# jlogan03/interpn

Hardware: AMD Instinct MI355X
Metric: Mpoints/sec (f64) per GPU + achieved HBM GB/s vs roofline, 3D linear-regular (higher is better)
Workload: dtype f64

## Files before the change

interpn_amd/csrc/abi_binned.hip:

```cpp
#include "abi_internal.h"

using namespace interpn;
using namespace interpn_abi;

namespace interpn_abi {


size_t bin_slice_points(const GridDesc& g) {
  const int lg = g.cfg.bin_slice_log2 >= 16 && g.cfg.bin_slice_log2 <= 27 ? g.cfg.bin_slice_log2 : 25;
  const size_t s = (size_t)1 << lg;
  return s < kBinSlicePoints ? s : kBinSlicePoints;
}

int binned_applies(const GridDesc& g, size_t npoints) {
  if (g.method != kCubic || !g.bricks || g.ndims < 2 || g.ndims > 4) return 0;
  if (g.cfg.binned == 0 || g.cfg.force_generic) return 1;
  const bool main11 = g.brick_step[0] == 1 && g.brick_step[1] == 1;
  const bool second = !main11 && g.bricks11 != nullptr;
  if (g.cfg.binned < 0) {
    if (g.ndims != 4 && g.ndims != 3) return 0;
    if (!main11 && !second) return 0;
    if (g.ndims == 3) return 0;
    if (main11) {
      unsigned nb[2];
      size_t table = 0;
      cubic_tile_geometry(g, 1, 1, nb, &table);
      if (table <= thresholds(g.cfg).binned_table_min) return 0;
    }
    if (npoints < thresholds(g.cfg).binned_points_min) return 1;
  }
  return 2;
}

interpn_hip_interp::BinSlot* take_bin_slot(interpn_hip_interp* h, size_t need, hipStream_t stream, bool may_alloc, int* why) {
  using Slot = interpn_hip_interp::BinSlot;
  std::unique_lock<std::mutex> lk(h->bin_mu);
  Slot* pick = nullptr;
  bool wait = false;
  for (auto& sl : h->bin_slots)
    if (!sl.busy && sl.bytes >= need && sl.recorded && sl.last_stream == stream) { pick = &sl; break; }
  if (!pick)
    for (auto& sl : h->bin_slots) {
      if (sl.busy || sl.bytes < need) continue;
      if (!sl.recorded) { pick = &sl; break; }
      const hipError_t q = hipEventQuery(sl.event);
      if (q == hipSuccess) { pick = &sl; break; }
      if (q != hipErrorNotReady) (void)hipGetLastError();
    }
  if (!pick && may_alloc && h->bin_slots.size() < interpn_hip_interp::kMaxBinSlots) {
    Slot sl;
    if (hipEventCreateWithFlags(&sl.event, hipEventDisableTiming) != hipSuccess) { (void)hipGetLastError(); *why = INTERPN_HIP_WHY_ALLOC_FAILED; return nullptr; }
    if (pool_alloc(h->device, &sl.scratch, need) != hipSuccess) {
      (void)hipGetLastError();
      (void)hipEventDestroy(sl.event);
      *why = INTERPN_HIP_WHY_ALLOC_FAILED;
      return nullptr;
    }
    sl.bytes = need;
    h->scratch_allocs.fetch_add(1);
    h->bin_slots.push_back(sl);
    pick = &h->bin_slots.back();
  }
  if (!pick) {
    for (auto& sl : h->bin_slots)
      if (!sl.busy && sl.bytes >= need && (!pick || sl.stamp < pick->stamp)) pick = &sl;
    wait = pick != nullptr;
  }
  if (!pick && may_alloc) {
    for (auto& sl : h->bin_slots)
      if (!sl.busy && (!pick || sl.stamp < pick->stamp)) pick = &sl;
    if (pick) {
      pick->busy = true;
      const bool recorded = pick->recorded;
      const hipEvent_t ev = pick->event;
      void* const old = pick->scratch;
      lk.unlock();
      bool freed = false;
      void* fresh = nullptr;
      bool ok = !recorded || hipEventSynchronize(ev) == hipSuccess;
      if (ok) {
        pool_free(h->device, old);
        freed = true;
        ok = pool_alloc(h->device, &fresh, need) == hipSuccess;
      }
      if (!ok) (void)hipGetLastError();
      lk.lock();
      if (freed) h->sampling.last_word = nullptr;
      pick->busy = false;
      if (!ok) {
        if (freed) { pick->scratch = nullptr; pick->bytes = 0; pick->recorded = false; }
        pick->totals_clean = false;
        pick->sweep_clean = false;
        *why = INTERPN_HIP_WHY_ALLOC_FAILED;
        return nullptr;
      }
      pick->scratch = fresh;
      pick->bytes = need;
      pick->totals_clean = false;
      pick->sweep_clean = false;
      pick->recorded = false;
      h->scratch_allocs.fetch_add(1);
    }
  }
  if (!pick) { *why = INTERPN_HIP_WHY_NO_SCRATCH; return nullptr; }
  if (wait && pick->recorded && pick->last_stream != stream &&
      hipStreamWaitEvent(stream, pick->event, 0) != hipSuccess) { (void)hipGetLastError(); *why = INTERPN_HIP_WHY_NO_SCRATCH; return nullptr; }
  if (!wait && pick->recorded && pick->last_stream != stream) (void)hipStreamWaitEvent(stream, pick->event, 0);
  pick->busy = true;
  pick->stamp = ++h->bin_uses;
  return pick;
}

void release_bin_slot(interpn_hip_interp* h, interpn_hip_interp::BinSlot* slot, hipStream_t stream, bool staged) {
  std::lock_guard<std::mutex> lk(h->bin_mu);
  if (hipEventRecord(slot->event, stream) == hipSuccess) {
    slot->recorded = true;
  } else {
    (void)hipGetLastError();
    (void)hipStreamSynchronize(stream);
    slot->recorded = false;
  }
  slot->last_stream = stream;
  slot->busy = false;
  slot->staged = staged;
}

int eval_device_binned(interpn_hip_interp* h, const void* const* obs, void* out, size_t npoints, hipStream_t stream,
                       unsigned flags, int* why) {
  const GridDesc& g = h->desc;
  *why = INTERPN_HIP_WHY_NONE;
  const int applies = binned_applies(g, npoints);
  if (applies < 2) { *why = applies ? INTERPN_HIP_WHY_SMALL_OR_OFF : INTERPN_HIP_WHY_NONE; return -1; }
  const bool main11 = g.brick_step[0] == 1 && g.brick_step[1] == 1;
  const bool second = !main11 && g.bricks11 != nullptr;
  GridDesc second_desc;
  const GridDesc* use = &g;
  if (second) {
    second_desc = g;
    second_desc.bricks = g.bricks11;
    second_desc.brick_step[0] = second_desc.brick_step[1] = 1;
    second_desc.brick_nb[0] = g.bricks11_nb[0];
    second_desc.brick_nb[1] = g.bricks11_nb[1];
    use = &second_desc;
  }
  BinPlan plan;
  bool column3_go = false;
  bool column = g.cfg.column != 0 && (second || main11) && cubic_column_applies(*use);
  const bool column3 = g.ndims == 3 && g.cfg.column != 0 && (second || main11) && cubic3_column_applies(*use);
  if (g.ndims == 3 && g.cfg.binned < 0 && !column3) { *why = INTERPN_HIP_WHY_NONE; return -1; }
  {
    const size_t slice_max0 = bin_slice_points(g);
    const size_t per_slice = npoints < slice_max0 ? npoints : slice_max0;
    ColumnPlan cp0;
    size_t per_bin_min = 2304;
// ... 161 lines not shown
  if (!h || !ms || n < 4) return INTERPN_HIP_ERR_INVALID_ARGUMENT;
  DeviceGuard guard(h->device);
  if (!guard.ok()) return INTERPN_HIP_ERR_NO_DEVICE;
  std::lock_guard<std::mutex> lk(h->bin_mu);
  const interpn_hip_interp::BinSlot* best = nullptr;
  for (const auto& sl : h->bin_slots)
    if (sl.staged && !sl.busy && (!best || sl.stamp > best->stamp)) best = &sl;
  if (!best) return INTERPN_HIP_ERR_INVALID_ARGUMENT;
  HIP_TRY(hipEventSynchronize(best->stage[4]));
  for (int k = 0; k < 4; ++k) {
    float f = 0.f;
    HIP_TRY(hipEventElapsedTime(&f, best->stage[k], best->stage[k + 1]));
    ms[k] = (double)f;
  }
  return INTERPN_HIP_OK;
}

int interpn_hip_reserve(interpn_hip_interp* h, size_t npoints, int nstreams) {
  if (!h || nstreams < 0) return INTERPN_HIP_ERR_INVALID_ARGUMENT;
  if ((size_t)nstreams > interpn_hip_interp::kMaxBinSlots) nstreams = (int)interpn_hip_interp::kMaxBinSlots;
  const GridDesc& g = h->desc;
  const bool sorts = binned_applies(g, npoints) >= 2, sweeps = sweep_applies(g, npoints) >= 2;
  if (npoints == 0 || nstreams == 0 || (!sorts && !sweeps)) return INTERPN_HIP_OK;
  DeviceGuard guard(h->device);
  if (!guard.ok()) return INTERPN_HIP_ERR_NO_DEVICE;
  const size_t slice_max = bin_slice_points(g);
  const size_t need = sorts ? bin_scratch_bytes(g, npoints < slice_max ? npoints : slice_max) : sweep_work_bytes();
  std::lock_guard<std::mutex> lk(h->bin_mu);
  int have = 0;
  for (auto& sl : h->bin_slots)
    if (sl.bytes >= need) ++have;
  for (auto& sl : h->bin_slots) {
    if (have >= nstreams) break;
    if (sl.bytes >= need || sl.busy) continue;
    if (sl.recorded) HIP_TRY(hipEventSynchronize(sl.event));
    pool_free(h->device, sl.scratch);
    h->sampling.last_word = nullptr;
    sl.scratch = nullptr;
    sl.bytes = 0;
    sl.totals_clean = false;
    sl.sweep_clean = false;
    sl.recorded = false;
    hipError_t e = pool_alloc(h->device, &sl.scratch, need);
    if (e != hipSuccess) { (void)hipGetLastError(); sl.scratch = nullptr; return INTERPN_HIP_ERR_OUT_OF_MEMORY; }
    sl.bytes = need;
    h->scratch_allocs.fetch_add(1);
    ++have;
  }
  while (have < nstreams && h->bin_slots.size() < interpn_hip_interp::kMaxBinSlots) {
    interpn_hip_interp::BinSlot sl;
    HIP_TRY(hipEventCreateWithFlags(&sl.event, hipEventDisableTiming));
    hipError_t e = pool_alloc(h->device, &sl.scratch, need);
    if (e != hipSuccess) { (void)hipGetLastError(); (void)hipEventDestroy(sl.event); return INTERPN_HIP_ERR_OUT_OF_MEMORY; }
    sl.bytes = need;
    h->scratch_allocs.fetch_add(1);
    h->bin_slots.push_back(sl);
    ++have;
  }
  return have >= nstreams ? INTERPN_HIP_OK : INTERPN_HIP_ERR_OUT_OF_MEMORY;
}

}
```

interpn_amd/csrc/abi_create.hip:

```cpp
#include "abi_internal.h"
#include "cubic_cell_record.h"

using namespace interpn;
using namespace interpn_abi;

namespace interpn_abi {

thread_local bool t_defer_tables = false;

int finish_create(interpn_hip_interp* h, const void* vals, size_t nvals, size_t elem, int vals_mem) {
  GridDesc& g = h->desc;
  {
    const DeviceProps dp = device_props(h->device);
    g.cfg.num_cus = dp.num_cus;
    g.cfg.num_xcds = dp.num_xcds;
    g.cfg.l2_bytes = dp.l2_bytes;
    g.cfg.lds_per_cu = dp.lds_per_cu;
    g.cfg.lds_per_wg = dp.lds_per_wg;
  }
  latch_env(g.cfg);
  g.nvals = nvals;
  if (vals_mem == INTERPN_HIP_MEM_DEVICE) {
    g.vals = vals;
  } else {
// ... 477 lines not shown
  const size_t elem = g.dtype == kF64 ? 8 : 4;
  hipError_t e = pool_alloc(dev, &h->vals_owned, g.nvals * elem);
  if (e == hipSuccess) e = hipMemcpyPeer(h->vals_owned, dev, src->desc.vals, src->device, g.nvals * elem);
  if (e == hipSuccess && src->desc.axis_image && g.axis_alloc_bytes) {
    e = pool_alloc(dev, &h->grids_owned, g.axis_alloc_bytes);
    if (e == hipSuccess) e = hipMemcpyPeer(h->grids_owned, dev, src->desc.axis_image, src->device, g.axis_alloc_bytes);
    if (e == hipSuccess) {
      g.axis_image = h->grids_owned;
      for (int d = 0; d < g.ndims; ++d) g.grid[d] = (const char*)h->grids_owned + g.axis_g_off[d];
    }
  }
  if (e != hipSuccess) {
    interpn_hip_destroy(h);
    return hip_fail(e);
  }
  st = finish_create(h, h->vals_owned, g.nvals, elem, INTERPN_HIP_MEM_DEVICE);
  if (st) {
    interpn_hip_destroy(h);
    return st;
  }
  *out = h;
  return INTERPN_HIP_OK;
}

int interpn_hip_elem_size(const interpn_hip_interp* h) { return h ? (h->desc.dtype == kF64 ? 8 : 4) : 0; }
int interpn_hip_ndims(const interpn_hip_interp* h) { return h ? h->desc.ndims : 0; }
int interpn_hip_device(const interpn_hip_interp* h) { return h ? h->device : -1; }

void interpn_hip_destroy(interpn_hip_interp* h) {
  if (!h) return;
  DeviceGuard guard(h->device);
  {
    std::lock_guard<std::mutex> lk(h->marks_mu);
    for (auto& m : h->marks) {
      if (hipEventSynchronize(m.event) != hipSuccess) { (void)hipGetLastError(); h->sync_device_at_destroy = true; }
      (void)hipEventDestroy(m.event);
    }
    h->marks.clear();
  }
  for (auto& l : h->lane)
    if (l.stream && hipStreamSynchronize(l.stream) != hipSuccess) { (void)hipGetLastError(); h->sync_device_at_destroy = true; }
  if (h->sync_device_at_destroy) (void)hipDeviceSynchronize();
  for (auto& l : h->lane) {
    if (l.stream) pool_return_kit(h->device, l.stream, l.flag_host);
    pool_free(h->device, l.flag_dev);
    pool_free(h->device, l.obs);
    pool_free(h->device, l.out);
  }
  pool_return_small(h->device, h->small_host);
  for (auto& sl : h->bin_slots) {
    if (sl.event) (void)hipEventDestroy(sl.event);
    for (hipEvent_t e : sl.stage)
      if (e) (void)hipEventDestroy(e);
    pool_free(h->device, sl.scratch);
  }
  pool_free(h->device, h->first_bad);
  pool_return_pinned_word(h->device, h->finish_word);
  pool_return_pinned_word(h->device, h->sampling.host);
  pool_free(h->device, h->grids_owned);
  pool_free(h->device, h->bricks_owned);
  pool_free(h->device, h->bricks11_owned);
  pool_free(h->device, h->sweep_owned);
  pool_free(h->device, h->vals_owned);
  delete h;
}

}
```

interpn_amd/csrc/abi_fields.hip:

```cpp
#include <climits>

#include "abi_internal.h"

using namespace interpn;
using namespace interpn_abi;

namespace {

struct DeferTables {
  explicit DeferTables(bool on) { t_defer_tables = on; }
  ~DeferTables() { t_defer_tables = false; }
};

long long env_number(const char* name, long long fallback) {
  const char* env = getenv(name);
  if (!env || !*env) return fallback;
  char* end = nullptr;
  const long long v = strtoll(env, &end, 0);
  return (end == env || *end != 0) ? fallback : v;
}

}

namespace interpn_abi {
// ... 281 lines not shown
        [&](int m, size_t prod) { return validate_rectilinear<T>(m, grids, grid_lens, ngrids, prod); },               \
        [&](const T* v, size_t prod, int dev, interpn_hip_interp** h) {                                               \
          return create_rectilinear<T>(method, grids, grid_lens, ngrids, v, prod, INTERPN_HIP_MEM_DEVICE,             \
                                       linearize_extrapolation, dev, h);                                              \
        });                                                                                                           \
  }
DEFINE_FIELDS(double, f64)
DEFINE_FIELDS(float, f32)

int interpn_hip_fields_eval_device(interpn_hip_fields* s, const void* const* obs, size_t nobs, void* out, size_t out_stride,
                                   size_t npoints, void* stream, unsigned flags, int* path_taken) {
  if (path_taken) *path_taken = INTERPN_HIP_FIELDS_PATH_PER_FIELD;
  if (!s || s->sub.empty() || (!obs && nobs)) return INTERPN_HIP_ERR_INVALID_ARGUMENT;
  if (flags & ~(unsigned)INTERPN_HIP_EVAL_NO_ALLOC) return INTERPN_HIP_ERR_INVALID_ARGUMENT;
  int st = validate_obs(s->sub[0]->desc, nullptr, nobs, npoints);
  if (st) return st;
  if (npoints == 0) return INTERPN_HIP_OK;
  if (!out || out_stride < npoints) return INTERPN_HIP_ERR_INVALID_ARGUMENT;
  for (size_t i = 0; i < nobs; ++i)
    if (!obs[i]) return INTERPN_HIP_ERR_INVALID_ARGUMENT;
  DeviceGuard guard(s->device);
  if (!guard.ok()) return INTERPN_HIP_ERR_NO_DEVICE;
  hipStream_t hs = static_cast<hipStream_t>(stream);
  const bool fused = columns_take_fused(s, npoints, hs, flags);
  st = eval_columns(s, fused, obs, out, out_stride, npoints, hs, flags);
  if (st == INTERPN_HIP_OK && fused && path_taken) *path_taken = INTERPN_HIP_FIELDS_PATH_FUSED;
  return st;
}

int interpn_hip_fields_finish(interpn_hip_fields* s, void* stream, uint64_t* first_bad_index) {
  if (!s || s->sub.empty()) return INTERPN_HIP_ERR_INVALID_ARGUMENT;
  const size_t count = s->per_field_pending ? s->nfields : 1;
  s->per_field_pending = false;
  int error = INTERPN_HIP_OK;
  uint64_t best = ~(uint64_t)0;
  for (size_t f = 0; f < count; ++f) {
    uint64_t bad = 0;
    const int st = interpn_hip_finish(s->sub[f], stream, &bad);
    if (st == s->sub[f]->desc.unrep_status) best = bad < best ? bad : best;
    else if (st != INTERPN_HIP_OK && error == INTERPN_HIP_OK) error = st;
  }
  if (error) return error;
  if (best != ~(uint64_t)0) {
    if (first_bad_index) *first_bad_index = best;
    return s->sub[0]->desc.unrep_status;
  }
  return INTERPN_HIP_OK;
}

int interpn_hip_fields_eval_host(interpn_hip_fields* s, const void* const* obs, const size_t* obs_lens, size_t nobs, void* out,
                                 size_t out_stride, size_t nout) {
  if (!s || s->sub.empty() || (!obs && nobs) || (!obs_lens && nobs)) return INTERPN_HIP_ERR_INVALID_ARGUMENT;
  int st = validate_obs(s->sub[0]->desc, obs_lens, nobs, nout);
  if (st) return st;
  if (nout == 0) return INTERPN_HIP_OK;
  if (!out || out_stride < nout) return INTERPN_HIP_ERR_INVALID_ARGUMENT;
  for (size_t i = 0; i < nobs; ++i)
    if (!obs[i]) return INTERPN_HIP_ERR_INVALID_ARGUMENT;
  DeviceGuard guard(s->device);
  if (!guard.ok()) return INTERPN_HIP_ERR_NO_DEVICE;
  const size_t elem = s->dtype == kF64 ? 8 : 4;
  const long long opt_chunk = s->sub[0]->desc.cfg.host_chunk;
  size_t chunk = opt_chunk >= 1 ? (size_t)opt_chunk : ((size_t)2 << 20);
  if (chunk > nout) chunk = nout;
  std::lock_guard<std::mutex> host_lock(s->host_mu);
  if (!s->stream) HIP_TRY(pool_take_kit(s->device, &s->stream, &s->kit_word));
// ... 187 lines not shown
```

interpn_amd/csrc/abi_host.hip:

```cpp
#include "abi_internal.h"

using namespace interpn;
using namespace interpn_abi;

namespace interpn_abi {

int ensure_lane(interpn_hip_interp* h, int which, size_t points) {
  interpn_hip_interp::HostLane& l = h->lane[which];
  if (l.points >= points && l.obs) return INTERPN_HIP_OK;
  const size_t elem = h->desc.dtype == kF64 ? 8 : 4;
  if (l.obs) { HIP_TRY(hipStreamSynchronize(l.stream)); pool_free(h->device, l.obs); l.obs = nullptr; }
  if (l.out) { pool_free(h->device, l.out); l.out = nullptr; }
  l.points = 0;
  if (!l.stream) HIP_TRY(pool_take_kit(h->device, &l.stream, &l.flag_host));
  HIP_TRY(pool_alloc(h->device, &l.obs, (size_t)h->desc.ndims * points * elem));
  HIP_TRY(pool_alloc(h->device, &l.out, points * elem));
  if (!l.flag_dev) {
    HIP_TRY(pool_alloc(h->device, (void**)&l.flag_dev, sizeof(unsigned long long)));
    HIP_TRY(hipMemsetAsync(l.flag_dev, 0xFF, sizeof(unsigned long long), l.stream));
  }
  l.points = points;
  return INTERPN_HIP_OK;
}

// ... 138 lines not shown
  }
  HostPipeline p;
  p.h = h;
  p.obs = obs;
  p.out = out;
  p.nout = nout;
  p.chunk = nout <= kPipelineChunkPoints ? nout : kPipelineChunkPoints;
  if (h->desc.cfg.host_chunk >= 1)
    p.chunk = (size_t)h->desc.cfg.host_chunk < nout ? (size_t)h->desc.cfg.host_chunk : nout;
  p.nchunks = (nout + p.chunk - 1) / p.chunk;
  int st = ensure_lane(h, 0, p.chunk);
  if (st) return st;
  if (p.nchunks > 1) {
    st = ensure_lane(h, 1, p.chunk);
    if (st) return st;
    std::thread helper([&p] { p.lane_main(1); });
    p.lane_main(0);
    helper.join();
  } else {
    p.checked[1] = ~(size_t)0;
    p.lane_main(0);
  }
  if (p.error) return p.error;
  if (p.fail_chunk != ~(size_t)0) {
    if (bad_index) *bad_index = p.fail_index;
    return h->desc.unrep_status;
  }
  return INTERPN_HIP_OK;
}

}

namespace {
__global__ void k_status_to_host(const unsigned long long* dev_word, unsigned long long* host_word) {
  const unsigned long long v = __hip_atomic_load(dev_word, __ATOMIC_RELAXED, __HIP_MEMORY_SCOPE_AGENT);
  __hip_atomic_store(host_word, v, __ATOMIC_RELEASE, __HIP_MEMORY_SCOPE_SYSTEM);
}
}

extern "C" {

int interpn_hip_finish(interpn_hip_interp* h, void* stream, uint64_t* first_bad_index) {
  if (!h) return INTERPN_HIP_ERR_INVALID_ARGUMENT;
  DeviceGuard guard(h->device);
  if (!guard.ok()) return INTERPN_HIP_ERR_NO_DEVICE;
  hipStream_t s = static_cast<hipStream_t>(stream);
  std::lock_guard<std::mutex> lk(h->finish_mu);
  if (!h->finish_word) {
    HIP_TRY(pool_take_pinned_word(h->device, &h->finish_word));
    void* dp = nullptr;
    if (hipHostGetDevicePointer(&dp, h->finish_word, 0) == hipSuccess) h->finish_word_dev = static_cast<unsigned long long*>(dp);
    else (void)hipGetLastError();
  }
  *(volatile unsigned long long*)h->finish_word = kWordPending;
  hipStreamCaptureStatus cs = hipStreamCaptureStatusNone;
  const bool by_kernel = h->finish_word_dev && h->desc.cfg.finish_kernel != 0 &&
                         hipStreamIsCapturing(s, &cs) == hipSuccess && cs == hipStreamCaptureStatusNone;
  if (by_kernel) {
    hipLaunchKernelGGL(k_status_to_host, dim3(1), dim3(1), 0, s, (const unsigned long long*)h->first_bad, h->finish_word_dev);
    HIP_TRY(hipGetLastError());
  } else {
    (void)hipGetLastError();
    HIP_TRY(hipMemcpyAsync(h->finish_word, h->first_bad, sizeof(unsigned long long), hipMemcpyDeviceToHost, s));
  }
  HIP_TRY(wait_status_word(s, h->finish_word));
  const unsigned long long word = *(volatile unsigned long long*)h->finish_word;
  if (word == kNoBadIndexHost) return INTERPN_HIP_OK;
  HIP_TRY(hipMemsetAsync(h->first_bad, 0xFF, sizeof(word), s));
  HIP_TRY(hipStreamSynchronize(s));
  const unsigned long long settled = *(volatile unsigned long long*)h->finish_word;
  if (settled == kNoBadIndexHost) return INTERPN_HIP_OK;
  if (first_bad_index) *first_bad_index = (uint64_t)settled;
  return h->desc.unrep_status;
}

int interpn_hip_eval_host(interpn_hip_interp* h, const void* const* obs, const size_t* obs_lens, size_t nobs,
                          void* out, size_t nout) {
  if (!h || (!obs && nobs) || (!obs_lens && nobs)) return INTERPN_HIP_ERR_INVALID_ARGUMENT;
  int st = validate_obs(h->desc, obs_lens, nobs, nout);
  if (st) return st;
  if (nout == 0) return INTERPN_HIP_OK;
  if (!out) return INTERPN_HIP_ERR_INVALID_ARGUMENT;
  for (size_t i = 0; i < nobs; ++i)
    if (!obs[i]) return INTERPN_HIP_ERR_INVALID_ARGUMENT;
  return eval_host_impl(h, obs, nobs, out, nout, nullptr);
}

#define ONESHOT_TAIL(T)                                                                         \
  st = interpn_hip_eval_host(h, reinterpret_cast<const void* const*>(obs), obs_lens, nobs, out, nout); \
  interpn_hip_destroy(h);                                                                       \
  return st;

#define ONESHOT_PRECHECK(METHOD, NDIMS, VALIDATE)                  \
  {                                                                \
    int pst = (VALIDATE);                                          \
    if (pst) return pst;                                           \
    GridDesc tmp;                                                  \
    tmp.method = (METHOD);                                         \
    tmp.ndims = (int)(NDIMS);                                      \
    if (!obs_lens && nobs) return INTERPN_HIP_ERR_INVALID_ARGUMENT; \
    pst = validate_obs(tmp, obs_lens, nobs, nout);                 \
    if (pst) return pst;                                           \
  }

#define DEFINE_ONESHOT(T, SUFFIX)                                                                             \
  int interpn_hip_linear_regular_##SUFFIX(const size_t* dims, size_t ndims, const T* starts, size_t nstarts, \
// ... 80 lines not shown
```

interpn_amd/csrc/abi_internal.h:

```cpp
#pragma once
#include <hip/hip_runtime.h>

#include <atomic>
#include <condition_variable>
#include <cctype>
#include <cmath>
#include <cstdint>
#include <cstdio>
#include <cstdlib>
#include <cstring>
#include <chrono>
#include <mutex>
#include <new>
#include <string>
#include <thread>
#include <unordered_map>
#include <vector>

#include "../../include/interpn_hip.h"
#include "interpn_host.h"

namespace interpn {
hipError_t launch_linear_grad(const GridDesc& g, const void* const* obs, void* out, void* const* grad, size_t npts,
                              unsigned long long* first_bad, hipStream_t stream);
// ... 52 lines not shown

hipError_t pool_alloc(int device, void** out, size_t bytes);
void pool_free(int device, void* p);
size_t pool_trim(int device);
hipError_t pool_take_kit(int device, hipStream_t* stream, unsigned long long** flag_host);
void pool_return_kit(int device, hipStream_t stream, unsigned long long* flag_host);
hipError_t pool_take_pinned_word(int device, unsigned long long** word);
void pool_return_pinned_word(int device, unsigned long long* word);
constexpr size_t kSmallPoints = 8192;
constexpr size_t kSmallBytes = (size_t)(8 + 1) * kSmallPoints * 8;

hipError_t pool_take_small(int device, void** buf);
void pool_return_small(int device, void* buf);
struct DeviceProps { int num_cus = 256, num_xcds = 8; long long l2_bytes = 4 << 20, lds_per_cu = 160 << 10, lds_per_wg = 64 << 10; };
DeviceProps device_props(int device);
int device_num_cus(int device);

}

struct interpn_hip_interp {
  interpn::GridDesc desc;
  int device = 0;
  void* vals_owned = nullptr;
  void* grids_owned = nullptr;
  void* bricks_owned = nullptr;
  void* bricks11_owned = nullptr;
  void* sweep_owned = nullptr;
  unsigned long long* first_bad = nullptr;
  unsigned long long* finish_word = nullptr;
  unsigned long long* finish_word_dev = nullptr;
  std::mutex finish_mu;
  std::mutex host_mu;
  static constexpr size_t kMaxMarks = 16;
  struct StreamMark { hipStream_t stream; hipEvent_t event; };
  std::mutex marks_mu;
  std::vector<StreamMark> marks;
  bool sync_device_at_destroy = false;
  struct HostLane {
    size_t points = 0;
    void* obs = nullptr;
    void* out = nullptr;
    unsigned long long* flag_dev = nullptr;
    unsigned long long* flag_host = nullptr;
    hipStream_t stream = nullptr;
  } lane[2];
  void* small_host = nullptr;
  void* small_dev = nullptr;
  static constexpr size_t kMaxBinSlots = 4;
  struct BinSlot {
    void* scratch = nullptr;
    size_t bytes = 0;
    hipEvent_t event = nullptr;
    bool recorded = false;
    bool busy = false;
    hipStream_t last_stream = nullptr;
    unsigned long long stamp = 0;
    bool totals_clean = false;
    bool sweep_clean = false;
    hipEvent_t stage[5] = {nullptr, nullptr, nullptr, nullptr, nullptr};
    bool staged = false;
  };
  std::mutex bin_mu;
  std::vector<BinSlot> bin_slots;
  unsigned long long bin_uses = 0;
  interpn_hip_interp() { bin_slots.reserve(kMaxBinSlots); }
  std::atomic<long long> evals_binned{0}, evals_in_place{0}, evals_sweep{0}, scratch_allocs{0};
  struct SweepSampling {
    unsigned long long* host = nullptr;
    unsigned* host_dev = nullptr;
    unsigned seq = 0, seen = 0;
    int streak = 0;
    int streak_coherent = 0;
    int skipped = 0;
    const void* last_word = nullptr;
  } sampling;
};

struct interpn_hip_fields {
  int device = 0;
  int dtype = interpn::kF64;
  int ndims = 0;
  size_t nfields = 0;
  size_t field_stride = 0;
  size_t field_elems = 0;
  int per_line = 0;
  size_t lines = 0;
// ... 103 lines not shown
extern thread_local bool t_defer_tables;
int finish_create(interpn_hip_interp* h, const void* vals, size_t nvals, size_t elem, int vals_mem);
template <typename T>
int create_regular(int method, const size_t* dims, size_t ndims, const T* starts, size_t nstarts, const T* steps,
                   size_t nsteps, const T* vals, size_t nvals, int vals_mem, int linearize, int device,
                   interpn_hip_interp** handle);
template <typename T>
int create_rectilinear(int method, const T* const* grids, const size_t* grid_lens, size_t ngrids, const T* vals,
                       size_t nvals, int vals_mem, int linearize, int device, interpn_hip_interp** handle);
template <typename T>
int create_one_dim(int method, int kind, T start, T step, const T* grid, size_t ngrid, const T* vals, size_t nvals,
                   int vals_mem, int device, interpn_hip_interp** handle);

inline size_t align_up(size_t v, size_t a) { return (v + a - 1) / a * a; }

inline bool stream_capturing(hipStream_t stream) {
  hipStreamCaptureStatus cs = hipStreamCaptureStatusNone;
  if (hipStreamIsCapturing(stream, &cs) != hipSuccess) { (void)hipGetLastError(); return true; }
  return cs != hipStreamCaptureStatusNone;
}

inline int fail_sequence(interpn_hip_interp* h, hipError_t err, int st) {
  (void)hipGetLastError();
  std::lock_guard<std::mutex> lk(h->marks_mu);
  h->sync_device_at_destroy = true;
  return err != hipSuccess ? hip_fail(err) : st;
}

hipError_t launch_any(const GridDesc& g, const void* const* obs, void* out, size_t npts,
                      unsigned long long* first_bad, hipStream_t stream);
void mark_stream(interpn_hip_interp* h, hipStream_t stream);
constexpr size_t kHostChunkPoints = (size_t)4 << 20;

constexpr unsigned long long kWordPending = 0xFFFFFFFFFFFFFFFEull;
hipError_t wait_status_word(hipStream_t s, const unsigned long long* word);

int binned_applies(const GridDesc& g, size_t npoints);
interpn_hip_interp::BinSlot* take_bin_slot(interpn_hip_interp* h, size_t need, hipStream_t stream, bool may_alloc, int* why);
void release_bin_slot(interpn_hip_interp* h, interpn_hip_interp::BinSlot* slot, hipStream_t stream, bool staged);

interpn_hip_interp::BinSlot* take_slot_captured(interpn_hip_interp* h, size_t need, hipStream_t stream);
void release_slot_captured(interpn_hip_interp* h, interpn_hip_interp::BinSlot* slot);
void claim_slot(interpn_hip_interp* h, interpn_hip_interp::BinSlot* slot);
int reserve_slots(interpn_hip_interp* h, size_t need, int nstreams);
int lattice_plan_args(size_t elem_size, int method, size_t ndims, const size_t* dims, const size_t* axis_lens, int* n,
                      interpn::LatticeShape* s, bool* indexable);
int lattice_make_shape(const void* const* axes, const size_t* axis_lens, size_t naxes, interpn::LatticeShape* s);
int validate_lattice(const interpn_hip_interp* h, const void* const* axes, const size_t* axis_lens, size_t naxes, const void* out,
                     interpn::LatticeShape* s, bool* empty);
interpn::LatticePlan lattice_plan_for(const GridDesc& g, const interpn::LatticeShape& s);
size_t lattice_scratch_need(const GridDesc& g, const interpn::LatticeShape& s, const interpn::LatticePlan& p);
size_t lattice_reserve_need(const GridDesc& g, const interpn::LatticeShape& s);
int lattice_device(interpn_hip_interp* h, const interpn::LatticeShape& s, void* out, hipStream_t stream, unsigned flags, int* path_taken);
constexpr size_t kExpandSliceBytes = (size_t)64 << 20;
constexpr size_t kExpandSliceMin = (size_t)1 << 16;

int ensure_sub_tables(interpn_hip_fields* s);

hipError_t launch_grad(const GridDesc& g, const void* const* obs, void* out, void* const* grad, size_t npts,
                       unsigned long long* first_bad, hipStream_t stream);

int eval_device_sweep(interpn_hip_interp* h, const void* const* obs, void* out, size_t npoints, hipStream_t stream,
                      unsigned flags, int* why);

int ensure_lane(interpn_hip_interp* h, int which, size_t points);
int eval_host_impl(interpn_hip_interp* h, const void* const* obs, size_t nobs, void* out, size_t nout, size_t* bad_index);

}
```

interpn_amd/csrc/abi_lattice.hip:

```cpp
#include "abi_internal.h"
#include "lattice.h"

using namespace interpn;
using namespace interpn_abi;

namespace interpn_abi {

using Slot = interpn_hip_interp::BinSlot;

Slot* take_slot_captured(interpn_hip_interp* h, size_t need, hipStream_t stream) {
  std::lock_guard<std::mutex> lk(h->bin_mu);
  Slot* pick = nullptr;
  for (auto& sl : h->bin_slots) {
    if (sl.busy || sl.bytes < need) continue;
    if (!pick || sl.last_stream == stream) pick = &sl;
  }
  if (pick) {
    pick->busy = true;
    pick->stamp = ++h->bin_uses;
  }
  return pick;
}

void release_slot_captured(interpn_hip_interp* h, Slot* slot) {
  std::lock_guard<std::mutex> lk(h->bin_mu);
  slot->busy = false;
}

void claim_slot(interpn_hip_interp* h, Slot* slot) {
  std::lock_guard<std::mutex> lk(h->bin_mu);
  slot->totals_clean = false;
  slot->sweep_clean = false;
  slot->staged = false;
  const unsigned char* word = static_cast<const unsigned char*>(h->sampling.last_word);
  const unsigned char* base = static_cast<const unsigned char*>(slot->scratch);
  if (word && word >= base && word < base + slot->bytes) h->sampling.last_word = nullptr;
}

int reserve_slots(interpn_hip_interp* h, size_t need, int nstreams) {
  std::lock_guard<std::mutex> lk(h->bin_mu);
  int have = 0;
  for (auto& sl : h->bin_slots)
    if (sl.bytes >= need) ++have;
  for (auto& sl : h->bin_slots) {
    if (have >= nstreams) break;
    if (sl.bytes >= need || sl.busy) continue;
    if (sl.recorded) HIP_TRY(hipEventSynchronize(sl.event));
    pool_free(h->device, sl.scratch);
    h->sampling.last_word = nullptr;
    sl.scratch = nullptr;
    sl.bytes = 0;
    sl.totals_clean = false;
    sl.sweep_clean = false;
    sl.recorded = false;
    if (pool_alloc(h->device, &sl.scratch, need) != hipSuccess) { (void)hipGetLastError(); sl.scratch = nullptr; return INTERPN_HIP_ERR_OUT_OF_MEMORY; }
    sl.bytes = need;
    h->scratch_allocs.fetch_add(1);
    ++have;
  }
  while (have < nstreams && h->bin_slots.size() < interpn_hip_interp::kMaxBinSlots) {
    Slot sl;
    HIP_TRY(hipEventCreateWithFlags(&sl.event, hipEventDisableTiming));
    if (pool_alloc(h->device, &sl.scratch, need) != hipSuccess) { (void)hipGetLastError(); (void)hipEventDestroy(sl.event); return INTERPN_HIP_ERR_OUT_OF_MEMORY; }
    sl.bytes = need;
    h->scratch_allocs.fetch_add(1);
    h->bin_slots.push_back(sl);
    ++have;
  }
  return have >= nstreams ? INTERPN_HIP_OK : INTERPN_HIP_ERR_OUT_OF_MEMORY;
}

}

namespace {

constexpr size_t kHostChunkPointsLattice = (size_t)1 << 25;

}

// ... 253 lines not shown
```

interpn_amd/csrc/abi_launch.hip:

```cpp
#include "abi_internal.h"

using namespace interpn;
using namespace interpn_abi;

namespace interpn_abi {

template <typename T>
hipError_t launch(const GridDesc& g, const T* const* obs, T* out, size_t npts, unsigned long long* first_bad,
                  hipStream_t stream) {
  if (npts == 0) return hipSuccess;
  if (g.method == kNearest) return launch_nearest<T>(g, obs, out, npts, first_bad, stream);
  if (g.cfg.force_generic || !fast_path(g)) return launch_generic<T>(g, obs, out, npts, first_bad, stream);
  if (g.method == kLinear)
    return g.kind == kRegular ? launch_linear_regular<T>(g, obs, out, npts, first_bad, stream)
                              : launch_linear_rectilinear<T>(g, obs, out, npts, first_bad, stream);
  return g.kind == kRegular ? launch_cubic_regular<T>(g, obs, out, npts, first_bad, stream)
                            : launch_cubic_rectilinear<T>(g, obs, out, npts, first_bad, stream);
}

hipError_t launch_any(const GridDesc& g, const void* const* obs, void* out, size_t npts,
                      unsigned long long* first_bad, hipStream_t stream) {
  if (is_one_dim(g.method)) return launch_one_dim(g, obs[0], out, npts, first_bad, stream);
  if (g.bricks && npts && g.method == kCubic && !g.cfg.force_generic) {
    if (g.dtype == kF64)
      return launch_cubic_brick<double>(g, reinterpret_cast<const double* const*>(obs), static_cast<double*>(out),
                                        npts, first_bad, stream);
    return launch_cubic_brick<float>(g, reinterpret_cast<const float* const*>(obs), static_cast<float*>(out), npts,
                                     first_bad, stream);
  }
  if (g.bricks && npts && g.ndims == 1 && g.method == kLinear && g.rec1_buckets && !g.cfg.force_generic) {
    if (g.dtype == kF64)
      return launch_linear1_records<double>(g, reinterpret_cast<const double* const*>(obs), static_cast<double*>(out), npts, stream);
    return launch_linear1_records<float>(g, reinterpret_cast<const float* const*>(obs), static_cast<float*>(out), npts, stream);
  }
  if (g.bricks && npts && g.ndims == 2 && !g.cfg.force_generic) {
    if (g.dtype == kF64)
      return launch_linear2_brick<double>(g, reinterpret_cast<const double* const*>(obs), static_cast<double*>(out),
                                          npts, first_bad, stream);
    return launch_linear2_brick<float>(g, reinterpret_cast<const float* const*>(obs), static_cast<float*>(out), npts,
                                       first_bad, stream);
  }
  if (g.bricks && npts && !g.cfg.force_generic) {
    if (g.dtype == kF64)
      return launch_linear_brick<double>(g, reinterpret_cast<const double* const*>(obs), static_cast<double*>(out),
                                         npts, first_bad, stream);
    return launch_linear_brick<float>(g, reinterpret_cast<const float* const*>(obs), static_cast<float*>(out), npts,
                                      first_bad, stream);
  }
  if (g.dtype == kF64)
    return launch<double>(g, reinterpret_cast<const double* const*>(obs), static_cast<double*>(out), npts, first_bad, stream);
  return launch<float>(g, reinterpret_cast<const float* const*>(obs), static_cast<float*>(out), npts, first_bad, stream);
}

hipError_t wait_status_word(hipStream_t s, const unsigned long long* word) {
  const volatile unsigned long long* w = word;
  const auto t0 = std::chrono::steady_clock::now();
  for (unsigned spin = 0;; ++spin) {
    if (*w != kWordPending) return hipSuccess;
#if defined(__x86_64__) || defined(__i386__)
    __builtin_ia32_pause();
#endif
    if ((spin & 255u) == 255u && std::chrono::steady_clock::now() - t0 > std::chrono::microseconds(200)) break;
  }
  return hipStreamSynchronize(s);
}

void mark_stream(interpn_hip_interp* h, hipStream_t stream) {
  hipStreamCaptureStatus cs = hipStreamCaptureStatusNone;
  if (hipStreamIsCapturing(stream, &cs) != hipSuccess) {
    (void)hipGetLastError();
    std::lock_guard<std::mutex> lk(h->marks_mu);
    h->sync_device_at_destroy = true;
    return;
  }
  std::lock_guard<std::mutex> lk(h->marks_mu);
  if (cs != hipStreamCaptureStatusNone) {
    h->sync_device_at_destroy = true;
    return;
  }
  for (auto& m : h->marks)
    if (m.stream == stream) {
      if (hipEventRecord(m.event, stream) != hipSuccess) { (void)hipGetLastError(); h->sync_device_at_destroy = true; }
      return;
    }
  hipEvent_t ev = nullptr;
  if (h->marks.size() >= interpn_hip_interp::kMaxMarks ||
      hipEventCreateWithFlags(&ev, hipEventDisableTiming) != hipSuccess) {
    (void)hipGetLastError();
    h->sync_device_at_destroy = true;
    return;
  }
  if (hipEventRecord(ev, stream) != hipSuccess) {
    (void)hipGetLastError();
    (void)hipEventDestroy(ev);
    h->sync_device_at_destroy = true;
    return;
  }
  h->marks.push_back({stream, ev});
}

}
```

interpn_amd/csrc/abi_sweep.hip:

```cpp
#include "abi_internal.h"

using namespace interpn;
using namespace interpn_abi;

namespace interpn {

int sweep_applies(const GridDesc& g, size_t npts) {
  if (g.method == kNearest) return nearest_sweep_applies(g, npts);
  if (g.method == kCubic) return cubic_sweep_applies(g, npts);
  if (g.ndims == 2) return linear2_sweep_applies(g, npts);
  return linear3_sweep_applies(g, npts);
}

hipError_t launch_sweep(const GridDesc& g, const void* const* obs, void* out, size_t npts, unsigned long long* first_bad,
                        void* work, hipStream_t stream) {
  if (!work || npts == 0) return hipErrorInvalidValue;
  if (g.method == kNearest) return launch_nearest_sweep(g, obs, out, npts, first_bad, work, stream);
  if (g.method == kCubic) return launch_cubic_sweep(g, obs, out, npts, first_bad, work, stream);
  if (g.ndims == 2) return launch_linear2_sweep(g, obs, out, npts, first_bad, work, stream);
  return launch_linear3_sweep(g, obs, out, npts, first_bad, work, stream);
}

}

namespace interpn_abi {

namespace {

struct SampleChoice {
  bool sample = false;
  bool one_pass_only = false;
  unsigned* host_word = nullptr;
  unsigned seq = 0;
};

SampleChoice choose_sample(interpn_hip_interp* h, const interpn_hip_interp::BinSlot* slot, size_t npoints) {
  const GridDesc& g = h->desc;
  SampleChoice c;
  c.sample = sweep_probe_applies(g) && npoints >= 256u * 64u;
  std::lock_guard<std::mutex> lk(h->bin_mu);
  interpn_hip_interp::SweepSampling& s = h->sampling;
  if (c.sample && g.cfg.sweep_probe == 2) {
    if (!s.host) {
      void* dp = nullptr;
      if (pool_take_pinned_word(h->device, &s.host) == hipSuccess && s.host &&
          hipHostGetDevicePointer(&dp, s.host, 0) == hipSuccess && dp) {
        *(volatile unsigned long long*)s.host = 0;
        s.host_dev = static_cast<unsigned*>(dp);
      } else {
        (void)hipGetLastError();
        s.host_dev = nullptr;
      }
    }
    if (s.host_dev) {
      const unsigned w = (unsigned)*(volatile unsigned long long*)s.host;
      if ((w >> 1) != s.seen && (w >> 1) != 0) {
        s.seen = w >> 1;
        s.streak = (w & 1u) ? 0 : s.streak + 1;
        s.streak_coherent = (w & 1u) ? s.streak_coherent + 1 : 0;
      }
      if ((s.streak >= 3 || s.streak_coherent >= 3) && s.skipped < 15) {
        ++s.skipped;
        c.sample = false;
        c.one_pass_only = s.streak < 3;
      } else {
        s.skipped = 0;
        s.seq = s.seq >= 0x7FFFFFFEu ? 1u : s.seq + 1u;
        c.host_word = s.host_dev;
        c.seq = s.seq;
      }
    }
  }
  s.last_word = c.sample ? static_cast<const unsigned char*>(slot->scratch) + sweep_probe_word_offset() : nullptr;
  return c;
}

}

int eval_device_sweep(interpn_hip_interp* h, const void* const* obs, void* out, size_t npoints, hipStream_t stream,
                      unsigned flags, int* why) {
  const GridDesc& g = h->desc;
  *why = INTERPN_HIP_WHY_NONE;
  const int applies = sweep_applies(g, npoints);
  if (applies < 2) { *why = applies ? INTERPN_HIP_WHY_SMALL_OR_OFF : INTERPN_HIP_WHY_NONE; return -1; }
  if (reinterpret_cast<uintptr_t>(out) % 16) { *why = INTERPN_HIP_WHY_MISALIGNED; return -1; }
  for (int d = 0; d < g.ndims; ++d)
    if (reinterpret_cast<uintptr_t>(obs[d]) % 16) { *why = INTERPN_HIP_WHY_MISALIGNED; return -1; }
  hipStreamCaptureStatus cs = hipStreamCaptureStatusNone;
  if (hipStreamIsCapturing(stream, &cs) != hipSuccess) { (void)hipGetLastError(); *why = INTERPN_HIP_WHY_CAPTURE; return -1; }
  if (cs != hipStreamCaptureStatusNone) { *why = INTERPN_HIP_WHY_CAPTURE; return -1; }
  interpn_hip_interp::BinSlot* slot = take_bin_slot(h, sweep_work_bytes(), stream, !(flags & INTERPN_HIP_EVAL_NO_ALLOC), why);
  if (!slot) return -1;
  hipError_t err = hipSuccess;
  if (!slot->sweep_clean) err = hipMemsetAsync(slot->scratch, 0, sweep_work_bytes(), stream);
  const SampleChoice c = choose_sample(h, slot, npoints);
  if (c.sample && err == hipSuccess) err = launch_sweep_probe(g, obs, npoints, slot->scratch, stream, c.host_word, c.seq);
  if (c.one_pass_only) {
    if (err == hipSuccess) {
      GridDesc gb = g;
      gb.launch_fat = true;
      err = launch_any(gb, obs, out, npoints, h->first_bad, stream);
      g.tag = gb.tag;
    }
  } else if (err == hipSuccess) {
    if (c.sample) {
      GridDesc gs = g;
      gs.sweep_gated = true;
      err = launch_sweep(gs, obs, out, npoints, h->first_bad, slot->scratch, stream);
      g.tag = gs.tag;
    } else {
      err = launch_sweep(g, obs, out, npoints, h->first_bad, slot->scratch, stream);
    }
  }
  if (c.sample && err == hipSuccess) {
    GridDesc gb = g;
    gb.launch_gate = reinterpret_cast<const unsigned*>(static_cast<const unsigned char*>(slot->scratch) + sweep_probe_word_offset());
    err = launch_any(gb, obs, out, npoints, h->first_bad, stream);
  }
  slot->sweep_clean = err == hipSuccess;
  slot->totals_clean = false;
  release_bin_slot(h, slot, stream, false);
  if (err != hipSuccess) {
    (void)hipGetLastError();
    return hip_fail(err);
  }
  return INTERPN_HIP_OK;
}

}
```

interpn_amd/csrc/interpn_host.h:

```cpp
#pragma once

#include <hip/hip_runtime.h>
#include <stddef.h>

#include <initializer_list>

namespace interpn {

enum Method : int { kLinear = 0, kCubic = 1, kNearest = 2 };
enum OneDimMethod : int { kLinear1D = 16, kLinearHoldLast1D = 17, kLeft1D = 18, kRight1D = 19, kNearest1D = 20 };
inline bool is_one_dim(int method) { return method >= kLinear1D && method <= kNearest1D; }
enum Kind : int { kRegular = 0, kRectilinear = 1 };
enum DType : int { kF64 = 0, kF32 = 1 };

struct LaunchConfig {
  int num_cus = 256;
  int num_xcds = 8;
  long long l2_bytes = 4ll << 20;
  long long lds_per_cu = 160ll << 10;
  long long lds_per_wg = 64ll << 10;
  int blocks_per_cu = 8;
  int iters_per_block = 0;
  int ppl = 0;
  int axis_regs = -1;
  int force_generic = 0;
  int generic_runtime = 0;
  int generic_vec = -1;
  int persistent = 0;
  int axis_lds_kb = -1;
  long long host_chunk = 0;
  int deal = 1;
  int binned = -1;
  int column = -1;
  int column_part = 0;
  int axis_records = 1;
  int stage_timing = 0;
  int bin_scramble = 0;
  int column_threads = 768;
  int column_groups = 1;
  int scatter_staged = 1;
  int column_coef = 1;
  int column_tail = 0x84;
  int column_keys = 1;
  int hist_wgs_per_cu = 4;
  int column_pad = -1;
  int column_cpp = 0;
  long long debug_stamps = 0;
  long long debug_stamps_bytes = 0;
  int bin_slice_log2 = 25;
  int sweep = -1;
  int finish_kernel = 0;
  int gated_iters = 4;
  int sweep_probe = 2;
  int lattice = -1;
  int points_path = 0;
  int points_load = 0;
  int points_store = 0;
  long long points_slice = 0;
  int sweep_period = 0;
};

struct KernelTag {
  const char* name = nullptr;
  int nargs = 0;
  int args[12] = {0};
  unsigned bool_mask = 0;
  void set(const char* nm, std::initializer_list<int> a, unsigned bools) {
    name = nm;
    nargs = 0;
    for (int v : a)
      if (nargs < 12) args[nargs++] = v;
    bool_mask = bools;
  }
};

struct GridDesc {
  const unsigned* launch_gate = nullptr;
  bool sweep_gated = false;
  bool launch_fat = false;
  int method = kLinear;
  int kind = kRegular;
  int dtype = kF64;
  int ndims = 0;
  int linearize = 0;
// ... 260 lines not shown
```

Measured before the change: 108,300.

## Defer slot event recording, drop per-call mark events, batch multi-field finish

```diff
diff --git a/interpn_amd/csrc/abi_binned.hip b/interpn_amd/csrc/abi_binned.hip
--- a/interpn_amd/csrc/abi_binned.hip
+++ b/interpn_amd/csrc/abi_binned.hip
@@ -32,16 +32,33 @@
   return 2;
 }
 
+bool settle_slot(interpn_hip_interp* h, interpn_hip_interp::BinSlot& sl) {
+  if (!sl.unmarked) return true;
+  hipStreamCaptureStatus cs = hipStreamCaptureStatusNone;
+  hipError_t e = hipStreamIsCapturing(sl.last_stream, &cs);
+  if (e == hipSuccess && cs != hipStreamCaptureStatusNone) return false;
+  if (e == hipSuccess) e = hipEventRecord(sl.event, sl.last_stream);
+  sl.unmarked = false;
+  sl.recorded = e == hipSuccess;
+  if (e != hipSuccess) {
+    (void)hipGetLastError();
+    if (hipDeviceSynchronize() != hipSuccess) (void)hipGetLastError();
+    std::lock_guard<std::mutex> lk(h->marks_mu);
+    h->sync_device_at_destroy = true;
+  }
+  return true;
+}
+
 interpn_hip_interp::BinSlot* take_bin_slot(interpn_hip_interp* h, size_t need, hipStream_t stream, bool may_alloc, int* why) {
   using Slot = interpn_hip_interp::BinSlot;
   std::unique_lock<std::mutex> lk(h->bin_mu);
   Slot* pick = nullptr;
   bool wait = false;
   for (auto& sl : h->bin_slots)
-    if (!sl.busy && sl.bytes >= need && sl.recorded && sl.last_stream == stream) { pick = &sl; break; }
+    if (!sl.busy && sl.bytes >= need && (sl.recorded || sl.unmarked) && sl.last_stream == stream) { pick = &sl; break; }
   if (!pick)
     for (auto& sl : h->bin_slots) {
-      if (sl.busy || sl.bytes < need) continue;
+      if (sl.busy || sl.bytes < need || !settle_slot(h, sl)) continue;
       if (!sl.recorded) { pick = &sl; break; }
       const hipError_t q = hipEventQuery(sl.event);
       if (q == hipSuccess) { pick = &sl; break; }
@@ -63,12 +80,12 @@
   }
   if (!pick) {
     for (auto& sl : h->bin_slots)
-      if (!sl.busy && sl.bytes >= need && (!pick || sl.stamp < pick->stamp)) pick = &sl;
+      if (!sl.busy && !sl.unmarked && sl.bytes >= need && (!pick || sl.stamp < pick->stamp)) pick = &sl;
     wait = pick != nullptr;
   }
   if (!pick && may_alloc) {
     for (auto& sl : h->bin_slots)
-      if (!sl.busy && (!pick || sl.stamp < pick->stamp)) pick = &sl;
+      if (!sl.busy && settle_slot(h, sl) && (!pick || sl.stamp < pick->stamp)) pick = &sl;
     if (pick) {
       pick->busy = true;
       const bool recorded = pick->recorded;
@@ -113,13 +130,8 @@
 
 void release_bin_slot(interpn_hip_interp* h, interpn_hip_interp::BinSlot* slot, hipStream_t stream, bool staged) {
   std::lock_guard<std::mutex> lk(h->bin_mu);
-  if (hipEventRecord(slot->event, stream) == hipSuccess) {
-    slot->recorded = true;
-  } else {
-    (void)hipGetLastError();
-    (void)hipStreamSynchronize(stream);
-    slot->recorded = false;
-  }
+  slot->unmarked = true;
+  slot->recorded = false;
   slot->last_stream = stream;
   slot->busy = false;
   slot->staged = staged;
@@ -347,7 +359,7 @@
     if (sl.bytes >= need) ++have;
   for (auto& sl : h->bin_slots) {
     if (have >= nstreams) break;
-    if (sl.bytes >= need || sl.busy) continue;
+    if (sl.bytes >= need || sl.busy || !settle_slot(h, sl)) continue;
     if (sl.recorded) HIP_TRY(hipEventSynchronize(sl.event));
     pool_free(h->device, sl.scratch);
     h->sampling.last_word = nullptr;
diff --git a/interpn_amd/csrc/abi_create.hip b/interpn_amd/csrc/abi_create.hip
--- a/interpn_amd/csrc/abi_create.hip
+++ b/interpn_amd/csrc/abi_create.hip
@@ -533,9 +533,12 @@
   DeviceGuard guard(h->device);
   {
     std::lock_guard<std::mutex> lk(h->marks_mu);
-    for (auto& m : h->marks) {
-      if (hipEventSynchronize(m.event) != hipSuccess) { (void)hipGetLastError(); h->sync_device_at_destroy = true; }
-      (void)hipEventDestroy(m.event);
+    for (hipStream_t m : h->marks) {
+      hipStreamCaptureStatus cs = hipStreamCaptureStatusNone;
+      if (hipStreamIsCapturing(m, &cs) != hipSuccess || cs != hipStreamCaptureStatusNone || hipStreamSynchronize(m) != hipSuccess) {
+        (void)hipGetLastError();
+        h->sync_device_at_destroy = true;
+      }
     }
     h->marks.clear();
   }
diff --git a/interpn_amd/csrc/abi_fields.hip b/interpn_amd/csrc/abi_fields.hip
--- a/interpn_amd/csrc/abi_fields.hip
+++ b/interpn_amd/csrc/abi_fields.hip
@@ -337,6 +337,12 @@
   if (!s || s->sub.empty()) return INTERPN_HIP_ERR_INVALID_ARGUMENT;
   const size_t count = s->per_field_pending ? s->nfields : 1;
   s->per_field_pending = false;
+  if (count > 1 && count <= (size_t)kMaxStatusWords) {
+    unsigned long long* words[kMaxStatusWords];
+    for (size_t f = 0; f < count; ++f) words[f] = s->sub[f]->first_bad;
+    const int st = finish_words(s->sub[0], static_cast<hipStream_t>(stream), words, (int)count, first_bad_index);
+    if (st >= 0) return st;
+  }
   int error = INTERPN_HIP_OK;
   uint64_t best = ~(uint64_t)0;
   for (size_t f = 0; f < count; ++f) {
diff --git a/interpn_amd/csrc/abi_host.hip b/interpn_amd/csrc/abi_host.hip
--- a/interpn_amd/csrc/abi_host.hip
+++ b/interpn_amd/csrc/abi_host.hip
@@ -194,19 +194,25 @@
 }
 
 namespace {
-__global__ void k_status_to_host(const unsigned long long* dev_word, unsigned long long* host_word) {
-  const unsigned long long v = __hip_atomic_load(dev_word, __ATOMIC_RELAXED, __HIP_MEMORY_SCOPE_AGENT);
+struct StatusWords {
+  const unsigned long long* word[interpn_abi::kMaxStatusWords];
+  int count;
+};
+__global__ void k_status_to_host(StatusWords w, unsigned long long* host_word) {
+  unsigned long long v = ~0ull;
+  for (int k = 0; k < w.count; ++k) {
+    const unsigned long long x = __hip_atomic_load(w.word[k], __ATOMIC_RELAXED, __HIP_MEMORY_SCOPE_AGENT);
+    v = x < v ? x : v;
+  }
   __hip_atomic_store(host_word, v, __ATOMIC_RELEASE, __HIP_MEMORY_SCOPE_SYSTEM);
 }
 }
 
-extern "C" {
-
-int interpn_hip_finish(interpn_hip_interp* h, void* stream, uint64_t* first_bad_index) {
-  if (!h) return INTERPN_HIP_ERR_INVALID_ARGUMENT;
+namespace interpn_abi {
+
+int finish_words(interpn_hip_interp* h, hipStream_t s, unsigned long long* const* words, int count, uint64_t* first_bad_index) {
   DeviceGuard guard(h->device);
   if (!guard.ok()) return INTERPN_HIP_ERR_NO_DEVICE;
-  hipStream_t s = static_cast<hipStream_t>(stream);
   std::lock_guard<std::mutex> lk(h->finish_mu);
   if (!h->finish_word) {
     HIP_TRY(pool_take_pinned_word(h->device, &h->finish_word));
@@ -214,26 +220,37 @@
     if (hipHostGetDevicePointer(&dp, h->finish_word, 0) == hipSuccess) h->finish_word_dev = static_cast<unsigned long long*>(dp);
     else (void)hipGetLastError();
   }
-  *(volatile unsigned long long*)h->finish_word = kWordPending;
   hipStreamCaptureStatus cs = hipStreamCaptureStatusNone;
-  const bool by_kernel = h->finish_word_dev && h->desc.cfg.finish_kernel != 0 &&
-                         hipStreamIsCapturing(s, &cs) == hipSuccess && cs == hipStreamCaptureStatusNone;
+  const hipError_t asked = hipStreamIsCapturing(s, &cs);
+  if (asked != hipSuccess) (void)hipGetLastError();
+  const bool by_kernel = h->finish_word_dev && h->desc.cfg.finish_kernel != 0 && count <= kMaxStatusWords && asked == hipSuccess &&
+                         cs == hipStreamCaptureStatusNone;
+  if (!by_kernel && count > 1) return -1;
   if (by_kernel) {
-    hipLaunchKernelGGL(k_status_to_host, dim3(1), dim3(1), 0, s, (const unsigned long long*)h->first_bad, h->finish_word_dev);
+    StatusWords w;
+    for (int k = 0; k < kMaxStatusWords; ++k) w.word[k] = words[k < count ? k : 0];
+    w.count = count;
+    hipLaunchKernelGGL(k_status_to_host, dim3(1), dim3(1), 0, s, w, h->finish_word_dev);
     HIP_TRY(hipGetLastError());
   } else {
-    (void)hipGetLastError();
-    HIP_TRY(hipMemcpyAsync(h->finish_word, h->first_bad, sizeof(unsigned long long), hipMemcpyDeviceToHost, s));
-  }
-  HIP_TRY(wait_status_word(s, h->finish_word));
+    HIP_TRY(hipMemcpyAsync(h->finish_word, words[0], sizeof(unsigned long long), hipMemcpyDeviceToHost, s));
+  }
+  HIP_TRY(hipStreamSynchronize(s));
   const unsigned long long word = *(volatile unsigned long long*)h->finish_word;
   if (word == kNoBadIndexHost) return INTERPN_HIP_OK;
-  HIP_TRY(hipMemsetAsync(h->first_bad, 0xFF, sizeof(word), s));
+  for (int k = 0; k < count; ++k) HIP_TRY(hipMemsetAsync(words[k], 0xFF, sizeof(word), s));
   HIP_TRY(hipStreamSynchronize(s));
-  const unsigned long long settled = *(volatile unsigned long long*)h->finish_word;
-  if (settled == kNoBadIndexHost) return INTERPN_HIP_OK;
-  if (first_bad_index) *first_bad_index = (uint64_t)settled;
+  if (first_bad_index) *first_bad_index = (uint64_t)word;
   return h->desc.unrep_status;
+}
+
+}
+
+extern "C" {
+
+int interpn_hip_finish(interpn_hip_interp* h, void* stream, uint64_t* first_bad_index) {
+  if (!h) return INTERPN_HIP_ERR_INVALID_ARGUMENT;
+  return finish_words(h, static_cast<hipStream_t>(stream), &h->first_bad, 1, first_bad_index);
 }
 
 int interpn_hip_eval_host(interpn_hip_interp* h, const void* const* obs, const size_t* obs_lens, size_t nobs,
diff --git a/interpn_amd/csrc/abi_internal.h b/interpn_amd/csrc/abi_internal.h
--- a/interpn_amd/csrc/abi_internal.h
+++ b/interpn_amd/csrc/abi_internal.h
@@ -108,9 +108,8 @@
   std::mutex finish_mu;
   std::mutex host_mu;
   static constexpr size_t kMaxMarks = 16;
-  struct StreamMark { hipStream_t stream; hipEvent_t event; };
   std::mutex marks_mu;
-  std::vector<StreamMark> marks;
+  std::vector<hipStream_t> marks;
   bool sync_device_at_destroy = false;
   struct HostLane {
     size_t points = 0;
@@ -128,6 +127,7 @@
     size_t bytes = 0;
     hipEvent_t event = nullptr;
     bool recorded = false;
+    bool unmarked = false;
     bool busy = false;
     hipStream_t last_stream = nullptr;
     unsigned long long stamp = 0;
@@ -297,12 +297,13 @@
 void mark_stream(interpn_hip_interp* h, hipStream_t stream);
 constexpr size_t kHostChunkPoints = (size_t)4 << 20;
 
-constexpr unsigned long long kWordPending = 0xFFFFFFFFFFFFFFFEull;
-hipError_t wait_status_word(hipStream_t s, const unsigned long long* word);
+constexpr int kMaxStatusWords = 32;
+int finish_words(interpn_hip_interp* h, hipStream_t s, unsigned long long* const* words, int count, uint64_t* first_bad_index);
 
 int binned_applies(const GridDesc& g, size_t npoints);
 interpn_hip_interp::BinSlot* take_bin_slot(interpn_hip_interp* h, size_t need, hipStream_t stream, bool may_alloc, int* why);
 void release_bin_slot(interpn_hip_interp* h, interpn_hip_interp::BinSlot* slot, hipStream_t stream, bool staged);
+bool settle_slot(interpn_hip_interp* h, interpn_hip_interp::BinSlot& slot);
 
 interpn_hip_interp::BinSlot* take_slot_captured(interpn_hip_interp* h, size_t need, hipStream_t stream);
 void release_slot_captured(interpn_hip_interp* h, interpn_hip_interp::BinSlot* slot);
diff --git a/interpn_amd/csrc/abi_lattice.hip b/interpn_amd/csrc/abi_lattice.hip
--- a/interpn_amd/csrc/abi_lattice.hip
+++ b/interpn_amd/csrc/abi_lattice.hip
@@ -44,7 +44,7 @@
     if (sl.bytes >= need) ++have;
   for (auto& sl : h->bin_slots) {
     if (have >= nstreams) break;
-    if (sl.bytes >= need || sl.busy) continue;
+    if (sl.bytes >= need || sl.busy || !settle_slot(h, sl)) continue;
     if (sl.recorded) HIP_TRY(hipEventSynchronize(sl.event));
     pool_free(h->device, sl.scratch);
     h->sampling.last_word = nullptr;
diff --git a/interpn_amd/csrc/abi_launch.hip b/interpn_amd/csrc/abi_launch.hip
--- a/interpn_amd/csrc/abi_launch.hip
+++ b/interpn_amd/csrc/abi_launch.hip
@@ -52,19 +52,6 @@
   return launch<float>(g, reinterpret_cast<const float* const*>(obs), static_cast<float*>(out), npts, first_bad, stream);
 }
 
-hipError_t wait_status_word(hipStream_t s, const unsigned long long* word) {
-  const volatile unsigned long long* w = word;
-  const auto t0 = std::chrono::steady_clock::now();
-  for (unsigned spin = 0;; ++spin) {
-    if (*w != kWordPending) return hipSuccess;
-#if defined(__x86_64__) || defined(__i386__)
-    __builtin_ia32_pause();
-#endif
-    if ((spin & 255u) == 255u && std::chrono::steady_clock::now() - t0 > std::chrono::microseconds(200)) break;
-  }
-  return hipStreamSynchronize(s);
-}
-
 void mark_stream(interpn_hip_interp* h, hipStream_t stream) {
   hipStreamCaptureStatus cs = hipStreamCaptureStatusNone;
   if (hipStreamIsCapturing(stream, &cs) != hipSuccess) {
@@ -78,25 +65,13 @@
     h->sync_device_at_destroy = true;
     return;
   }
-  for (auto& m : h->marks)
-    if (m.stream == stream) {
-      if (hipEventRecord(m.event, stream) != hipSuccess) { (void)hipGetLastError(); h->sync_device_at_destroy = true; }
-      return;
-    }
-  hipEvent_t ev = nullptr;
-  if (h->marks.size() >= interpn_hip_interp::kMaxMarks ||
-      hipEventCreateWithFlags(&ev, hipEventDisableTiming) != hipSuccess) {
-    (void)hipGetLastError();
+  for (hipStream_t m : h->marks)
+    if (m == stream) return;
+  if (h->marks.size() >= interpn_hip_interp::kMaxMarks) {
     h->sync_device_at_destroy = true;
     return;
   }
-  if (hipEventRecord(ev, stream) != hipSuccess) {
-    (void)hipGetLastError();
-    (void)hipEventDestroy(ev);
-    h->sync_device_at_destroy = true;
-    return;
-  }
-  h->marks.push_back({stream, ev});
+  h->marks.push_back(stream);
 }
 
 }
diff --git a/interpn_amd/csrc/abi_sweep.hip b/interpn_amd/csrc/abi_sweep.hip
--- a/interpn_amd/csrc/abi_sweep.hip
+++ b/interpn_amd/csrc/abi_sweep.hip
@@ -34,7 +34,7 @@
   unsigned seq = 0;
 };
 
-SampleChoice choose_sample(interpn_hip_interp* h, const interpn_hip_interp::BinSlot* slot, size_t npoints) {
+SampleChoice choose_sample(interpn_hip_interp* h, size_t npoints) {
   const GridDesc& g = h->desc;
   SampleChoice c;
   c.sample = sweep_probe_applies(g) && npoints >= 256u * 64u;
@@ -71,7 +71,7 @@
       }
     }
   }
-  s.last_word = c.sample ? static_cast<const unsigned char*>(slot->scratch) + sweep_probe_word_offset() : nullptr;
+  s.last_word = nullptr;
   return c;
 }
 
@@ -89,20 +89,28 @@
   hipStreamCaptureStatus cs = hipStreamCaptureStatusNone;
   if (hipStreamIsCapturing(stream, &cs) != hipSuccess) { (void)hipGetLastError(); *why = INTERPN_HIP_WHY_CAPTURE; return -1; }
   if (cs != hipStreamCaptureStatusNone) { *why = INTERPN_HIP_WHY_CAPTURE; return -1; }
+  const SampleChoice c = choose_sample(h, npoints);
+  if (c.one_pass_only) {
+    GridDesc gb = g;
+    gb.launch_fat = true;
+    const hipError_t e1 = launch_any(gb, obs, out, npoints, h->first_bad, stream);
+    g.tag = gb.tag;
+    if (e1 != hipSuccess) {
+      (void)hipGetLastError();
+      return hip_fail(e1);
+    }
+    return INTERPN_HIP_OK;
+  }
   interpn_hip_interp::BinSlot* slot = take_bin_slot(h, sweep_work_bytes(), stream, !(flags & INTERPN_HIP_EVAL_NO_ALLOC), why);
   if (!slot) return -1;
+  if (c.sample) {
+    std::lock_guard<std::mutex> lk(h->bin_mu);
+    h->sampling.last_word = static_cast<const unsigned char*>(slot->scratch) + sweep_probe_word_offset();
+  }
   hipError_t err = hipSuccess;
   if (!slot->sweep_clean) err = hipMemsetAsync(slot->scratch, 0, sweep_work_bytes(), stream);
-  const SampleChoice c = choose_sample(h, slot, npoints);
   if (c.sample && err == hipSuccess) err = launch_sweep_probe(g, obs, npoints, slot->scratch, stream, c.host_word, c.seq);
-  if (c.one_pass_only) {
-    if (err == hipSuccess) {
-      GridDesc gb = g;
-      gb.launch_fat = true;
-      err = launch_any(gb, obs, out, npoints, h->first_bad, stream);
-      g.tag = gb.tag;
-    }
-  } else if (err == hipSuccess) {
+  if (err == hipSuccess) {
     if (c.sample) {
       GridDesc gs = g;
       gs.sweep_gated = true;
diff --git a/interpn_amd/csrc/interpn_host.h b/interpn_amd/csrc/interpn_host.h
--- a/interpn_amd/csrc/interpn_host.h
+++ b/interpn_amd/csrc/interpn_host.h
@@ -49,7 +49,7 @@
   long long debug_stamps_bytes = 0;
   int bin_slice_log2 = 25;
   int sweep = -1;
-  int finish_kernel = 0;
+  int finish_kernel = 1;
   int gated_iters = 4;
   int sweep_probe = 2;
   int lattice = -1;
```

Result: faster. 109,600, median of 6 (+1.2%).
